# theori-io/nrsc5

Hardware: NVIDIA H100
Metric: cu8 I/Q Msamples/s (higher is better)
Workload: dtype u8/int16/f32

## Files before the change

### nrsc5_b200/csrc/common.cuh

```cuda
#pragma once
#include <cuda_runtime.h>
#include <stdint.h>

namespace nb {

constexpr int NFFT = 2048;
constexpr int NCP = 112;
constexpr int NSYM = NFFT + NCP;
constexpr int BLK = 32;
constexpr int NACQ = NSYM * (BLK + 1);
constexpr int LB0 = NFFT / 2 - 546;
constexpr int UB1 = NFFT / 2 + 546;
constexpr int PW = 19;
constexpr int MAXPART = 14;
constexpr int SIDE = MAXPART * PW + 1;
constexpr int NBINS = 2 * SIDE;
constexpr int PM_BLOCK = 23040;
constexpr int P1_LEN = 146176;
constexpr int P1_ENC = P1_LEN * 5 / 2;
constexpr int P1_VIT = P1_LEN * 3;
constexpr int P1_STEPS = P1_LEN + 64;
constexpr int PIDS_LEN = 80;
constexpr int P3_LEN = 4608;
constexpr int IV_N = 147456;
// ... 125 lines not shown
    int8_t *pm;
    short2 *ydec;
    float2 *acq_sums;
    float2 *tbuf;
    int8_t *vit_in;
    uint2 *vit_dec;
    uint32_t *p1_bits;
    uint2 *vspec, *vend;
    int *hstate, *tbend;
    uint32_t *v64_spec, *v64_end;
    int *v64_endstate;
    int8_t *px_ring[2];
    const uint32_t *iv_delay;
    const uint32_t *iv_delay_s;
    PxBufs xb[PX_GROUPS];
    uint8_t *log;
    const float *shape;
    const float2 *twid;
    const uint32_t *p1_lut;
    const uint8_t *pn;
    const uint32_t *pnw;
};

__device__ inline uint8_t *log_reserve(const DevPtrs &p, const EngineDims &d, int s, uint32_t type, uint32_t plen)
{
    StreamState &st = p.st[s];
    uint32_t need = 8 + ((plen + 3) & ~3u);
    if ((size_t)st.log_len + need > d.log_cap) {
        st.log_overflow = 1;
        return nullptr;
    }
    uint8_t *w = p.log + (size_t)s * d.log_cap + st.log_len;
    reinterpret_cast<uint32_t *>(w)[0] = type;
    reinterpret_cast<uint32_t *>(w)[1] = plen;
    st.log_len += need;
    return w + 8;
}

__device__ __forceinline__ void l2_enqueue(StreamState &st, int l2_on, unsigned off, unsigned lc, unsigned nbits)
{
    if (!l2_on) return;
    if (st.l2_n >= L2_QUEUE) {
        st.log_overflow = 1;
        return;
    }
    const int e = st.l2_n++;
    st.l2_off[e] = off;
    st.l2_lc[e] = lc;
    st.l2_nbits[e] = nbits;
// ... 39 lines not shown
```

### nrsc5_b200/csrc/engine.cu

```cuda
#include <cmath>
#include <cstdio>
#include <cstdlib>
#include <cstring>
#include <ctime>
#include <new>
#include <vector>

#include "../../include/nrsc5_b200.h"
#include "chan_feed.h"
#include "common.cuh"
#if defined(NB_EMU)
struct NvtxRange { explicit NvtxRange(const char *) {} };
#else
#include <nvtx3/nvToolsExt.h>
struct NvtxRange {
    explicit NvtxRange(const char *name) { nvtxRangePushA(name); }
    ~NvtxRange() { nvtxRangePop(); }
};
#endif
#include "rs.cuh"
#include "viterbi.cuh"
#include "viterbi_chunk.cuh"
#include "viterbi64.cuh"
#include "front.cuh"
// ... 129 lines not shown
    gf_tab_load(gf, t, P1_THREADS);
    if (t < 96) {
        unsigned v = frame ? __ldcg(frame + t) : 0;
        hdr[t] = (uint8_t)(__brev(v) >> 24);
    }
    __syncthreads();
    if (t < 32) {
        unsigned bit = 0;
        if (t < 24) {
            const unsigned i = 116176u + 1248u * t;
            const unsigned phys = (i & ~7u) + 7 - (i & 7);
            bit = ((p1_bit(bw, (int)phys) ^ (p.pnw[phys >> 5] >> (phys & 31))) & 1u) << (23 - t);
        }
        const unsigned pci = warp_xor(bit);
        const bool has_audio = (pci & 0xFFFFFC) != (0x3634CE & 0xFFFFFC);
        const int ok = has_audio ? rs8_fix_header_warp(gf, hdr, t) : 1;
        if (t == 0) {
            if (rec) *reinterpret_cast<float *>(rec) = (float)atomicAdd(&st.p1_errs, 0) / (float)P1_ENC;
            if (!ok) {
                if (st.state == ST_FINE && st.p1_lost_rec != 0xffffffffu) {
                    *reinterpret_cast<uint32_t *>(p.log + (size_t)s * d.log_cap + st.p1_lost_rec) = REC_LOST_SYNC;
                    st.state = ST_NONE;
                } else {
                    set_state(p, d, s, ST_NONE);
                }
            }
            if (st.p1_retry) st.p1_fallbacks++;
            st.p1_ready = 0;
            st.p1_slow = 0;
            st.p1_retry = 0;
            st.frames_done++;
        }
    }
}

__host__ __device__ inline VitcArgs p1_vitc_args(const DevPtrs &dp)
{
    VitcArgs a;
    a.vin = dp.vit_in;
    a.dec = dp.vit_dec;
    a.vspec = dp.vspec;
    a.vend = dp.vend;
    a.hstate = dp.hstate;
    a.tbend = dp.tbend;
    a.bitsw = dp.p1_bits;
    a.ready = &dp.st[0].p1_retry;
    a.slow = &dp.st[0].p1_slow;
// ... 954 lines not shown
static int publish_avail(nrsc5b_engine *e, int s, cudaStream_t on);

static int publish_pending(nrsc5b_engine *e, cudaStream_t on)
{
    for (int s = 0; s < e->dims.nstreams; s++)
        if (e->unpublished[s]) {
            int rc = publish_avail(e, s, on);
            if (rc) return rc;
            e->unpublished[s] = 0;
        }
    return 0;
}

static int publish_avail(nrsc5b_engine *e, int s, cudaStream_t on)
{
    if (e->avail_pos && (e->avail_pos & 4095) == 0) CK(cudaStreamSynchronize(on));
    long long *slot = e->avail_ring + (e->avail_pos++ & 4095);
    *slot = e->pushed[s];
    CK(cudaMemcpyAsync(reinterpret_cast<uint8_t *>(e->dp.st + s) + offsetof(StreamState, in_avail), slot, sizeof(*slot),
                       cudaMemcpyHostToDevice, on));
    return 0;
}

__global__ void k_trim_state(DevPtrs p, int s, long long drop, nbam::AmState *ast)
{
    p.st[s].start -= drop;
    p.st[s].in_avail -= 2 * drop;
    if (ast) ast[s].start -= drop;
}

static int trim_stream(nrsc5b_engine *e, int s)
{
    CK(cudaStreamSynchronize(e->copy_stream));
    CK(cudaStreamSynchronize(e->stream));
    StreamState st;
    CK(cudaMemcpy(&st, e->dp.st + s, sizeof(st), cudaMemcpyDeviceToHost));
    long long drop = (st.start - 64) & ~7LL;
    if (st.start < 72 || drop <= 0) return 0;
    const size_t off = 4 * (size_t)drop, have = 2 * (size_t)e->pushed[s];
    if (off >= have) return 0;
    const size_t rem = have - off;
    uint8_t *base = e->iq_owned + (size_t)s * e->dims.in_stride;
    if (!e->trim_scratch) {
        void *q = nullptr;
        if (cudaMalloc(&q, e->dims.in_stride) != cudaSuccess) return NRSC5B_ENOMEM;
        e->allocs.push_back(q);
// ... 125 lines not shown
    for (int s = 0; s < S; s++) e->pushed[s] += (long long)(nbytes / 2);
    e->direct_push = true;
    return NRSC5B_OK;
}

extern "C" int nrsc5b_push_cu8_device(nrsc5b_engine_t *e, int stream, const void *dev_buf, size_t nbytes)
{
    if (!e || stream < 0 || stream >= e->dims.nstreams || (nbytes & 3) || !e->iq_owned || e->am_ring) return NRSC5B_EINVAL;
    size_t off = (size_t)e->pushed[stream] * 2;
    if (off + nbytes > e->dims.in_stride) return NRSC5B_EFULL;
    CK(cudaMemcpyAsync(e->iq_owned + (size_t)stream * e->dims.in_stride + off, dev_buf, nbytes,
                       cudaMemcpyDeviceToDevice, e->stream));
    e->pushed[stream] += (long long)(nbytes / 2);
    e->direct_push = true;
    return publish_avail(e, stream, e->stream);
}

extern "C" int nrsc5b_attach_device_input(nrsc5b_engine_t *e, const void *dev_buf, size_t stride, size_t nbytes)
{
    if (!e || !dev_buf || (nbytes & 3) || nbytes > stride || e->am_ring) return NRSC5B_EINVAL;
    e->dp.iq = reinterpret_cast<const uint8_t *>(dev_buf);
    e->dims.in_stride = stride;
    e->direct_push = true;
    for (int s = 0; s < e->dims.nstreams; s++) {
        e->pushed[s] = (long long)(nbytes / 2);
        int rc = publish_avail(e, s, e->stream);
        if (rc) return rc;
    }
    return NRSC5B_OK;
}

int nbfeed_reserve(nrsc5b_engine_t *e, int device, int mode, const int *streams, int nch, long long nout, FeedTarget *t, long long *dst)
{
    if (!e || !t || !dst || nch <= 0 || nout < 0) return NRSC5B_EINVAL;
    if (e->cfg.mode != mode || !e->dims.cs16 || !e->iq_owned || e->dp.iq != e->iq_owned || device != e->cfg.device ||
        e->in_flight)
        return NRSC5B_EINVAL;
    const int S = e->dims.nstreams;
    if (!streams && nch > S) return NRSC5B_EINVAL;
    std::vector<uint8_t> seen(S, 0);
    for (int k = 0; k < nch; k++) {
        const int s = streams ? streams[k] : k;
        if (s < 0 || s >= S || seen[s]) return NRSC5B_EINVAL;
        seen[s] = 1;
    }
    const size_t need = 4 * (size_t)nout;
    bool full = false;
    for (int k = 0; k < nch; k++) {
        const int s = streams ? streams[k] : k;
        if ((size_t)e->pushed[s] * 2 + need <= e->dims.in_stride) continue;
        int rc = trim_stream(e, s);
// ... 932 lines not shown
```

### nrsc5_b200/csrc/front.cuh

```cuda
#pragma once
#include "pids_crc.cuh"
#include "common.cuh"
#include "fft.cuh"
#include "viterbi_pack.cuh"

namespace nb {

constexpr int FRONT_THREADS = 1024;
constexpr int TEAMS = FRONT_THREADS / 128;
constexpr int MAXREF = 15;
constexpr int IN_BYTES = 4 * NSYM + 28 + 16 + 16;
constexpr int IN_STRIDE = 8704;
constexpr int ACQ_TILE = 4096;

__device__ int g_dbg;

__constant__ int c_compat_mode[64];
__constant__ unsigned c_pn80[3];
__constant__ short c_bp_tap[32];

__device__ __forceinline__ float2 cmulf(float2 a, float2 b)
{
    return make_float2(a.x * b.x - a.y * b.y, a.x * b.y + a.y * b.x);
}
__device__ __forceinline__ float2 cexp_j(float a)
{
    float s, c;
    sincosf(a, &s, &c);
    return make_float2(c, s);
}

__device__ __forceinline__ int partitions_per_band(int psmi)
{
    switch (c_compat_mode[psmi & 63]) {
    case 2: return 11;
    case 3: return 12;
    case 5: case 6: case 11: return 14;
    default: return 10;
    }
}

__device__ void set_state(const DevPtrs &p, const EngineDims &d, int s, int ns)
{
    StreamState &st = p.st[s];
    if (st.state == ns) return;
    if (st.state == ST_FINE) log_reserve(p, d, s, REC_LOST_SYNC, 0);
    if (ns == ST_FINE) {
        float fo = (float)(((double)st.prev_angle - 2 * M_PI * st.cfo) * 744187.5 / (2 * M_PI * NFFT));
        uint8_t *w = log_reserve(p, d, s, REC_SYNC, 8);
        if (w) {
            reinterpret_cast<float *>(w)[0] = fo;
            reinterpret_cast<int *>(w)[1] = st.psmi;
        }
    }
    st.state = ns;
}

constexpr int DEMOD_RUN = 17;
constexpr int TEAM_SMEM = IN_STRIDE + NSYM * (int)sizeof(short2);
struct DemodSmem {
    float2 buf[TEAMS][TEAM_SMEM / sizeof(float2)];
};
static_assert(FFT_SMEM_ELEMS * sizeof(float2) <= TEAM_SMEM && TEAM_SMEM % 16 == 0, "a team's FFT buffer");
static_assert(DEMOD_RUN * FFT_THREADS >= NSYM && DEMOD_RUN % 2 == 1, "a symbol's runs");
struct PrepSmem {
    uint32_t words[ACQ_TILE + 40];
    short2 ytile[ACQ_TILE + 32];
    float2 sums[NSYM];
    float red_mag[FRONT_THREADS];
    int red_idx[FRONT_THREADS];
    float2 red_v[FRONT_THREADS];
};
// ... 35 lines not shown
    float wred[FRONT_THREADS / 32][2];
    float fb_w[2][MAXREF], fb_xy[2][MAXREF + 1];
    float4 rowc[EQ_ROWS];
    int ref_ok[2 * MAXREF], ref_bc[2 * MAXREF], ref_psmi[2 * MAXREF];
    bool px_on[2];
    long long px_T[2];
    uint8_t *soft_w;
    int do_search;
};
struct BlockSet {
    int samperr;
    int ok;
    float prev_angle, angle;
    float theta;
    float2 phase0, phase;
};
struct FrontSmem {
    float2 tw[FFT_TW];
    float2 nco[NSYM];
    float2 symphase[BLK];
    BlockSet blk;
    float2 zref[BLK][ZS];
    uint8_t ref_plan[128];
    union {
        DemodSmem demod;
        PrepSmem prep;
        Acq1Smem acq1;
        SyncSmem sync;
        PidsSmem pidsq[16];
    } u;
};

__device__ void pids_decode_warp(const DevPtrs &p, const EngineDims &d, int s, int e, PidsSmem &sm, int lane)
{
    const StreamState &st = p.st[s];
    const int bc = st.pids_bc[e];
    const int8_t *pmall = p.pm + (size_t)s * 16 * PM_BLOCK;
    const int8_t PMV[20] = { 10, 2, 18, 6, 14, 8, 16, 0, 12, 4, 11, 3, 19, 7, 15, 9, 17, 1, 13, 5 };
    for (int o = lane; o < PIDS_LEN * 3; o += 32) {
        int8_t v = 0;
        if (o % 6 != 5) {
            unsigned i = (unsigned)bc * 200 + (unsigned)(o - o / 6);
            unsigned part = (unsigned)PMV[i % 20];
            unsigned block = i / 200;
            unsigned k = (i / 20) % 10 + P1_ENC / 320;
            unsigned row = (k * 11) % 32, col = (k * 11 + k / 288) % 36;
            v = pmall[(block * 32 + row) * 720 + part * 36 + col];
        }
        sm.vit[o] = v;
    }
    __syncwarp();
    const int l = lane & 15;
    VitHalf<false> vh;
    vh.init(l);
    vitc_run<false>(vh, sm.vit, PIDS_LEN, PIDS_LEN + 64, 0, PIDS_LEN + 64, 0, sm.dec, lane < 16, l);
    __syncwarp();
    int v = (short)(vh.E & 0xffff), state = 2 * l;
    const int w1 = (short)(vh.O & 0xffff);
// ... 6 lines not shown
    for (int o = 8; o; o >>= 1) {
        const int ov = __shfl_xor_sync(0xffffffffu, v, o, 16), oi = __shfl_xor_sync(0xffffffffu, state, o, 16);
        if (ov > v || (ov == v && oi < state)) { v = ov; state = oi; }
    }
    if (lane == 0) {
        uint8_t pk[10];
        for (int i = 0; i < 10; i++) pk[i] = 0;
        for (int q = PIDS_LEN + 63; q >= 0; q--) {
            if (q >= 32 && q < 32 + PIDS_LEN) {
                const int i = q - 32;
                const int bit = ((state >> 5) & 1) ^ (int)((c_pn80[i >> 5] >> (i & 31)) & 1u);
                pk[i >> 3] |= (uint8_t)(bit << (7 - (i & 7)));
            }
            state = vitc_prev_head(state, sm.dec, q);
        }
        if (st.pids_rec[e] != 0xffffffffu) {
            uint8_t *w = p.log + (size_t)s * d.log_cap + st.pids_rec[e];
            for (int i = 0; i < 10; i++) w[i] = pk[i];
            w[10] = (uint8_t)pids_crc12_ok(pk);
        }
    }
}

__device__ void front_pids_flush(const DevPtrs &p, const EngineDims &d, int s, PidsSmem *sm, int t)
{
    StreamState &st = p.st[s];
    const int n = st.pids_pending, warp = t >> 5;
    if (warp < n) pids_decode_warp(p, d, s, warp, sm[warp], t & 31);
    __syncthreads();
    if (t == 0) st.pids_pending = 0;
}

constexpr int ACQ_RUN = 5;
static_assert(ACQ_RUN * FRONT_THREADS >= ACQ_TILE + 31, "a tile's runs");
template <int RUN>
__device__ __forceinline__ void acq_tile_input(const EngineDims &d, const uint32_t *words, short2 *ytile, const StreamState &st,
                                               int i0, int L, int t)
{
    const int kb = i0 == 0 ? 31 : 0;
    if (t < kb) ytile[t] = make_short2(st.bp_hist[t][0], st.bp_hist[t][1]);
    const int n = L + 31 - kb;
    if (d.cs16) {
        for (int k = kb + t; k < L + 31; k += FRONT_THREADS) {
            const uint32_t w = words[k + 7];
            ytile[k] = make_short2((short)(w & 0xffff), (short)(w >> 16));
        }
    } else if (RUN * t < n) {
        const int k = kb + min(RUN * t, n - RUN);
        halfband_run<RUN>(words + k, ytile + k);
    }
}
// ... 30 lines not shown
    double sn, cs;
    sincos((double)theta * (double)(NSYM * sym), &sn, &cs);
    symphase[sym] = cmul(phase0, make_float2((float)cs, (float)sn));
}

__device__ __forceinline__ void block_setup(BlockSet &b, const StreamState &st)
{
    const int adj = NSYM / 2 - b.samperr;
    float angle = b.prev_angle;
    angle = (float)((double)angle - 2 * M_PI * st.cfo);
    const float pre = (float)(-adj) * angle / (float)NFFT;
    const float2 ph = cmulf(st.phase, cexp_j(pre));
    const float theta = angle / (float)NFFT;
    double sn, cs;
    sincos((double)theta * (double)(NSYM * BLK), &sn, &cs);
    const float2 pe = cmulf(ph, make_float2((float)cs, (float)sn));
    const float nrm = sqrtf(pe.x * pe.x + pe.y * pe.y);
    b.angle = angle;
    b.theta = theta;
    b.phase0 = ph;
    b.phase = make_float2(pe.x / nrm, pe.y / nrm);
}

__device__ __forceinline__ void sync_adjust(const DevPtrs &p, int s, int adj, int t)
{
    if (adj == 0) return;
    float *cp = p.cphase + (size_t)s * NFFT;
    for (int i = t; i < SIDE; i += FRONT_THREADS) {
        const int bl = LB0 + i, bu = UB1 - i;
        cp[bl] = (float)((double)cp[bl] - (double)(adj * (bl - NFFT / 2) * 2) * M_PI / NFFT);
        cp[bu] = (float)((double)cp[bu] - (double)(adj * (bu - NFFT / 2) * 2) * M_PI / NFFT);
    }
}

__device__ __forceinline__ void block_commit(const DevPtrs &p, const EngineDims &d, int s, const BlockSet &b, int state_in)
{
    StreamState &st = p.st[s];
    st.phase0 = b.phase0;
    st.theta = b.theta;
    st.blk_samperr = b.samperr;
    st.blk_state_in = state_in;
    st.phase = b.phase;
    uint8_t *w = log_reserve(p, d, s, REC_BLOCK, 32);
    if (w) {
        int *wi = reinterpret_cast<int *>(w);
        float *wf = reinterpret_cast<float *>(w);
        wi[0] = state_in; wi[1] = b.samperr; wf[2] = b.angle; wf[3] = b.phase0.x; wf[4] = b.phase0.y; wi[5] = st.cfo;
        wi[6] = (int)(unsigned)(st.start & 0xffffffffLL);
        wi[7] = (int)(st.start >> 32);
    }
}

__device__ int front_prep_begin(const DevPtrs &p, const EngineDims &d, int s, int t)
{
    StreamState &st = p.st[s];
    __shared__ int sh_active;
    if (t == 0) {
        if (st.force_state >= 0) {
            set_state(p, d, s, st.force_state);
            st.force_state = -1;
        }
        const long long avail = *reinterpret_cast<volatile long long *>(&st.in_avail);
        int act = avail >= 2 * (st.start + NACQ);
        if (act && st.state == ST_FINE) {
            const int need = px_need_of(c_compat_mode[st.psmi & 63]);
            if (need & ~d.px_enabled) {
                atomicOr(&p.ctl->px_need, (unsigned)need);
                act = 0;
            }
        }
        st.active = act;
        sh_active = act ? (st.state == ST_FINE ? 1 : 2) : 0;
        if (act) atomicAdd(&p.ctl->progress, 1ull);
    }
    __syncthreads();
    const int mode = sh_active;
    __syncthreads();
    return mode;
}

__device__ void front_acq_tiles(const DevPtrs &p, const EngineDims &d, int s, PrepSmem &sm, int t, int rank, int nranks)
{
// ... 79 lines not shown
                }
            }
            __syncthreads();
        }
        if (t == 0) {
            const float2 w = cmulf(sm.red_v[0], cexp_j(-st.prev_angle));
            const float angle_diff = atan2f(w.y, w.x);
            const float factor = (st.prev_angle != 0.0f) ? 0.25f : 1.0f;
            const float angle = st.prev_angle + (angle_diff * factor);
            st.prev_angle = angle;
            b.prev_angle = angle;
            b.samperr = (sm.red_idx[0] + NSYM - 15) % NSYM;
            if (st.state == ST_NONE) st.state = ST_COARSE;
        }
    } else if (t == 0) {
        b.samperr = NSYM / 2 + st.samperr;
        st.samperr = 0;
        const float angle = st.prev_angle + (-st.angle);
        st.angle = 0;
        st.prev_angle = angle;
        b.prev_angle = angle;
    }
    __syncthreads();
    sync_adjust(p, s, NSYM / 2 - b.samperr, t);
    if (t == 0) {
        block_setup(b, st);
        block_commit(p, d, s, b, state_in);
    }
    __syncthreads();
    fill_nco(p, nco, b.theta, t);
    if (t >= FRONT_THREADS - BLK) fill_symphase(symphase, b.theta, b.phase0, t - (FRONT_THREADS - BLK));
    __syncthreads();
}

__device__ bool front_prep_single(const DevPtrs &p, const EngineDims &d, int s, Acq1Smem &sm, float2 *nco, float2 *symphase,
                                  BlockSet &b, int t)
{
    StreamState &st = p.st[s];
    __shared__ int sh_active;
    if (t == 0) {
        const int fs = st.force_state;
        const long long avail = *reinterpret_cast<volatile long long *>(&st.in_avail);
        const long long start = st.start;
        const int psmi = st.psmi;
        int state = st.state;
        if (fs >= 0) {
            set_state(p, d, s, fs);
            st.force_state = -1;
            state = fs;
        }
        int act = avail >= 2 * (start + NACQ);
        if (act && state == ST_FINE) {
            const int need = px_need_of(c_compat_mode[psmi & 63]);
            if (need & ~d.px_enabled) {
                atomicOr(&p.ctl->px_need, (unsigned)need);
                act = 0;
            }
        }
        st.active = act;
        sh_active = act ? (state == ST_FINE && b.ok ? 2 : 1) : 0;
        b.ok = 0;
        if (act) atomicAdd(&p.ctl->progress, 1ull);
    } else {
        fill_nco(p, nco, b.theta, t - 1, FRONT_THREADS - 1);
        if (t >= FRONT_THREADS - BLK) fill_symphase(symphase, b.theta, b.phase0, t - (FRONT_THREADS - BLK));
    }
    __syncthreads();
    if (!sh_active) return false;
    if (sh_active == 2) {
        sync_adjust(p, s, NSYM / 2 - b.samperr, t);
        if (t == 0) {
            st.samperr = 0;
            st.angle = 0;
            st.prev_angle = b.prev_angle;
            block_commit(p, d, s, b, ST_FINE);
        }
        return true;
    }

    const uint8_t *iq = p.iq + (size_t)s * d.in_stride;
    const int state_in = st.state;
    if (state_in != ST_FINE) {
        const long long start = st.start;
        constexpr int NT = BLK + 1;
        static_assert(NACQ == NT * NSYM, "the window is whole tiles");
        const int woff = (int)((start - 38) & 3);
        static_assert(NSYM % 4 == 0, "tiles start at the same word phase");
        const int nvec = (woff + NSYM + 38 + 3) / 4;
        auto fetch = [&](int T) {
            const long long w0 = start + (long long)T * NSYM - 38;
            const long long w0a = w0 & ~3LL;
            uint4 *dst = reinterpret_cast<uint4 *>(sm.words[T & 1]);
            for (int v = t; v < nvec; v += FRONT_THREADS) {
                const long long a = w0a + 4 * v;
                if (a >= 0) {
#if defined(NB_EMU)
                    dst[v] = *reinterpret_cast<const uint4 *>(iq + 4 * a);
#else
// ... 68 lines not shown
                }
            }
            __syncthreads();
        }
        if (t == 0) {
            const float2 w = cmulf(sm.red_v[0], cexp_j(-st.prev_angle));
            const float angle_diff = atan2f(w.y, w.x);
            const float factor = (st.prev_angle != 0.0f) ? 0.25f : 1.0f;
            const float angle = st.prev_angle + (angle_diff * factor);
            st.prev_angle = angle;
            b.prev_angle = angle;
            b.samperr = (sm.red_idx[0] + NSYM - 15) % NSYM;
            if (st.state == ST_NONE) st.state = ST_COARSE;
        }
    } else if (t == 0) {
        b.samperr = NSYM / 2 + st.samperr;
        st.samperr = 0;
        const float angle = st.prev_angle + (-st.angle);
        st.angle = 0;
        st.prev_angle = angle;
        b.prev_angle = angle;
    }
    __syncthreads();
    sync_adjust(p, s, NSYM / 2 - b.samperr, t);
    if (t == 0) {
        block_setup(b, st);
        block_commit(p, d, s, b, state_in);
    }
    __syncthreads();
    fill_nco(p, nco, b.theta, t);
    if (t >= FRONT_THREADS - BLK) fill_symphase(symphase, b.theta, b.phase0, t - (FRONT_THREADS - BLK));
    __syncthreads();
    return true;
}

__device__ __forceinline__ float2 sample_q15(short2 h)
{
    const float sc = 1.0f / 32767.0f;
    return make_float2((float)h.x * sc, (float)h.y * -sc);
}

__device__ void front_demod(const DevPtrs &p, const EngineDims &d, int s, int sym, DemodSmem &sm, const float2 *nco,
                            const float2 *symphase, const float2 *tw, float2 (*zref)[ZS], const uint8_t *ref_plan,
                            int half, int tl, long long start, int samperr)
{
    float2 *buf = sm.buf[half];
    uint8_t *in = reinterpret_cast<uint8_t *>(buf);
    const int bar = 1 + half;
    const long long base = start + samperr + (long long)NSYM * sym;
    const long long b0 = 4 * base - 28;
// ... 55 lines not shown

    float2 *dst = p.bins + ((size_t)s * BLK + sym) * NBINS;
    const unsigned plan = ref_plan[tl];
    float2 *zp = zref[sym] + (plan & 31u);
    const unsigned pk = plan >> 5;
    auto put = [&](int c, float2 v, unsigned k) {
        dst[c] = v;
        if (pk == k) *zp = v;
    };
#pragma unroll
    for (int h = 0; h < 2; h++) {
        const int q = tl + 128 * h;
        if (q >= 222) put(q - 222, cmul(out[h][5], sp), 4 * h);
        if (q <= 232) put(q + 34, cmul(out[h][6], sp), 4 * h + 1);
        if (q >= 24) put(q + 243, cmul(out[h][1], sp), 4 * h + 2);
        if (q <= 34) put(q + 499, cmul(out[h][2], sp), 4 * h + 3);
    }
}

__device__ __forceinline__ int ref_bin(int slot)
{
    return slot < MAXREF ? LB0 + PW * slot : UB1 - PW * (slot - MAXREF);
}

__device__ __forceinline__ float atan2_short(float y, float x)
{
    const float ax = fabsf(x), ay = fabsf(y);
    const float mx = fmaxf(ax, ay), mn = fminf(ax, ay);
    const float t = mx > 0.f ? __fdividef(mn, mx) : 0.f;
    const float z = t * t;
    float p = 0.0028340641874819994f;
    p = __fmaf_rn(p, z, -0.016005029901862144f);
    p = __fmaf_rn(p, z, 0.042587608098983765f);
    p = __fmaf_rn(p, z, -0.07495445758104324f);
    p = __fmaf_rn(p, z, 0.10636754333972931f);
    p = __fmaf_rn(p, z, -0.14202570915222168f);
    p = __fmaf_rn(p, z, 0.19992484152317047f);
    p = __fmaf_rn(p, z, -0.3333306610584259f);
    p = __fmaf_rn(p, z, 1.0f);
    float r = p * t;
    if (ay > ax) r = 1.57079637f - r;
    if (x < 0.f) r = 3.14159274f - r;
    return copysignf(r, y);
}

__device__ __forceinline__ void costas_row(float2 *z, float *phs, int zs, float &cfreq, float &cphase, int cfo, float alpha, float beta, bool FAST)
// ... 71 lines not shown
    }
    return -1;
}

__device__ __forceinline__ float half_pi_wrap(float a, float b)
{
    float dd = a - b;
    while ((double)dd > M_PI / 2) dd = (float)((double)dd - M_PI);
    while ((double)dd < -M_PI / 2) dd = (float)((double)dd + M_PI);
    return dd;
}

__device__ __forceinline__ int8_t soft_demap(float x, float mult)
{
    const float v = fmaxf(fminf(x, 1.0f), -1.0f) * mult;
    int r = __float2int_rz(v);
    const float f = v - (float)r;
    if (f >= 0.5f) r++;
    else if (f <= -0.5f) r--;
    return (int8_t)r;
}

template <bool CL>
__device__ void front_sync(const DevPtrs &p, const EngineDims &d, int s, SyncSmem &sm, float2 (*zref)[ZS], BlockSet &b, int t)
{
    StreamState &st = p.st[s];
    float *cfreq = p.cfreq + (size_t)s * NFFT;
    float *cphase = p.cphase + (size_t)s * NFFT;
    float2 *bins = p.bins + (size_t)s * BLK * NBINS;
    auto ldbin = [](const float2 *q) -> float2 { return CL ? __ldcg(q) : *q; };
    const float loop_bw = 0.05f, damping = 0.70710678f;
    const float denom = 1 + (2 * damping * loop_bw) + (loop_bw * loop_bw);
    const float alpha = (4 * damping * loop_bw) / denom, beta = (4 * loop_bw * loop_bw) / denom;

    int ppb = partitions_per_band(st.psmi);
    int nref = ppb + 1;
    long long sy0 = clock64();
    const bool sy_on = st.state == ST_FINE;
    auto sylap = [&](int k) {
        if (t == 0 && sy_on) {
            const long long c1 = clock64();
            st.sy_cyc[k] += (unsigned long long)(c1 - sy0);
            sy0 = c1;
        }
    };
    auto stage_eq = [&](int first, int stride) {
        const int rows = min(ppb, EQ_MAXPART) * (PW - 1), rows2 = 2 * rows;
        const int dn = stride / rows2, dr = stride - dn * rows2;
        int n = first / rows2, r = first - n * rows2;
#pragma unroll 4
        for (; n < BLK;) {
            const int sb = r >= rows, rr = sb ? r - rows : r;
            const int i = rr / (PW - 1);
            const int ci = sb == 0 ? rr + i + 1 : (NBINS - PW) + rr - (2 * PW - 1) * i;
            sm.eq[r][n] = ldbin(&bins[(size_t)n * NBINS + ci]);
            r += dr;
            n += dn;
            if (r >= rows2) { r -= rows2; n++; }
        }
    };
    const bool pre_staged = st.state == ST_FINE && !(g_dbg & 1);
    if (CL) {
        for (int i = t; i < ZS * BLK; i += FRONT_THREADS) {
            const int slot = i & (ZS - 1), n = i / ZS;
            const int ii = slot < MAXREF ? slot : slot - MAXREF;
            if (slot < 2 * MAXREF && ii < nref) zref[n][slot] = ldbin(&bins[(size_t)n * NBINS + compact_of_bin(ref_bin(slot))]);
        }
        __syncthreads();
    }
    sylap(0);
    if (t < 2 * MAXREF) {
        const int i = t < MAXREF ? t : t - MAXREF;
        if (i < nref) {
            const int b = ref_bin(t);
            float f = cfreq[b], ph = cphase[b];
            costas_row(&zref[0][t], &sm.phs[0][t], ZS, f, ph, 0, alpha, beta, !(g_dbg & 2));
            cfreq[b] = f;
            cphase[b] = ph;
            sm.cfq[t] = f;
            float sum = 0;
            for (int n = 0; n < BLK; n++) sum += fabsf(zref[n][t].x);
            sm.smag[t] = sum / BLK;
        }
    } else if (t >= 32 && pre_staged) {
        stage_eq(t - 32, FRONT_THREADS - 32);
    }
    __syncthreads();
    sylap(1);

    if (st.state == ST_COARSE) {
        if (t < 2 * MAXREF) {
            const int i = t < MAXREF ? t : t - MAXREF;
            sm.ref_ok[t] = 0;
            if (i < nref) {
                const float2 *z = &zref[0][t];
                const unsigned rsid = (unsigned)(30 - i) & 3;
                bool ok = true;
                unsigned raw = 0;
                for (int n = 0; n < BLK; n++) {
                    const int nbit = needle_bit(n, rsid);
                    const int pos = z[n * ZS].x > 0 ? 1 : 0;
// ... 8 lines not shown
            }
        }
        __syncthreads();
        if (t == 0) {
            unsigned good = 0;
            for (int r = 0; r < 2 * MAXREF; r++)
                if (sm.ref_ok[r]) good++;
            sm.do_search = 0;
            if (good >= 4) {
                int mbc = -1, mps = -1;
                for (int v = 0; v < 16; v++) {
                    unsigned nbc = 0, nps = 0;
                    for (int r = 0; r < 2 * MAXREF; r++) {
                        if (!sm.ref_ok[r]) continue;
                        nbc += sm.ref_bc[r] == v;
                        nps += sm.ref_psmi[r] == v;
                    }
                    if (nbc > good / 2) mbc = v;
                    if (nps > good / 2) mps = v;
                }
                if (mbc >= 0 && mps >= 0) {
                    st.bc = mbc;
                    st.psmi = mps;
                    set_state(p, d, s, ST_FINE);
                    l2_enqueue(st, d.l2, 0u, 0, 0);
                    st.started_pm = 0;
                    st.px_total[0] = st.px_total[1] = 0;
                    st.px_started[0] = st.px_started[1] = 0;
                }
            } else if (st.cfo_wait == 0) {
                sm.do_search = 1;
            } else {
                st.cfo_wait--;
            }
        }
        __syncthreads();
        if (sm.do_search) {
            for (int i = t; i < ZS * BLK; i += FRONT_THREADS) {
                const int slot = i & (ZS - 1), n = i / ZS;
                const int ii = slot < MAXREF ? slot : slot - MAXREF;
                if (slot < 2 * MAXREF && ii < nref) bins[(size_t)n * NBINS + compact_of_bin(ref_bin(slot))] = zref[n][slot];
            }
            for (int i = t; i < 76 * 22; i += FRONT_THREADS) sm.srch.offs[i / 22][i % 22] = -1;
            __syncthreads();
            constexpr int SB_BINS = 2 * PW * 2 + 10 * PW;
            constexpr int NSB = 2 * SB_BINS;
            float2 *snap = p.tbuf + (size_t)s * NACQ;
            float *sphs = reinterpret_cast<float *>(p.ydec + (size_t)s * NACQ);
            float fs[4], phsn[4];
            int cfo_of[4], nq = 0, ci = -1, b = 0;
            if (t < NSB) {
                const int upper = t >= SB_BINS;
                b = upper ? (UB1 - 10 * PW - 2 * PW) + (t - SB_BINS) : (LB0 - 2 * PW) + t;
                ci = compact_of_bin(b);
                float f = cfreq[b], ph = cphase[b];
                int ref_i[4];
                for (int step = 0; step <= 10; step++) {
                    const int i = upper ? step : 10 - step;
                    const int cfo = upper ? b - UB1 + PW * i : b - LB0 - PW * i;
                    if (cfo >= -2 * PW && cfo < 2 * PW && nq < 4) {
                        ref_i[nq] = i;
                        cfo_of[nq] = cfo;
                        nq++;
                    }
                }
                for (int q = 0; q < nq; q++) {
// ... 31 lines not shown
                if (win < (1 << 20)) {
                    st.keep_extra = ((BLK - sm.srch.verdict[win + 2 * PW]) % BLK) * NSYM;
                    st.cfo += win;
                    st.cfo_wait = 8;
                }
            }
            __syncthreads();
            if (t < NSB) {
                const int win = sm.srch.winner;
                int q = -1;
                for (int k = 0; k < nq; k++)
                    if (cfo_of[k] <= win) q = k;
                if (q >= 0) {
                    cfreq[b] = fs[q];
                    cphase[b] = phsn[q];
                    if (ci >= 0) {
                        const float2 *row = snap + (size_t)q * BLK * NSB + t;
                        for (int n = 0; n < BLK; n++) bins[(size_t)n * NBINS + ci] = row[(size_t)n * NSB];
                    }
                }
            }
        }
        __syncthreads();
    }

    if (st.state == ST_FINE) {
        for (int i = t; i < 2 * MAXREF * BLK; i += FRONT_THREADS) {
            const int slot = i >> 5, n = i & 31;
            const int ii = slot < MAXREF ? slot : slot - MAXREF;
            if (ii < nref) sm.eph[slot][n] = cexp_j(sm.phs[n][slot]);
        }
        const int bc = st.bc;
        int8_t *pm = p.pm + ((size_t)s * 16 + bc) * PM_BLOCK;
        const int rows = min(ppb, EQ_MAXPART) * (PW - 1), rows2 = 2 * rows;
        for (int r = t; r < rows2; r += FRONT_THREADS) {
            const int sb = r >= rows, rr = sb ? r - rows : r;
            const int i = rr / (PW - 1), k = rr - i * (PW - 1) + 1;
            int slot_lo, slot_hi;
            if (sb == 0) { slot_lo = i; slot_hi = i + 1; }
            else { slot_lo = MAXREF + i + 1; slot_hi = MAXREF + i; }
            sm.rowc[r] = make_float4((float)k * sm.smag[slot_hi], (float)(PW - k) * sm.smag[slot_lo],
                                     __int_as_float(slot_hi), __int_as_float(slot_lo));
        }
        sylap(2);
        if (!pre_staged) stage_eq(t, FRONT_THREADS);
        const int cm = c_compat_mode[st.psmi & 63];
// ... 130 lines not shown
                samperr = (float)((double)(samperr / (float)(ppb * 2) * (float)NFFT / (float)PW) * inv_2pi);
                for (int i = 0; i <= ppb; i++) {
                    float x;
                    x = (float)(LB0 + PW * i - NFFT / 2);
                    angle += sm.cfq[i]; sum_xy += sm.fb_xy[0][i]; sum_x2 += x * x;
                    x = (float)(UB1 - PW * i - NFFT / 2);
                    angle += sm.cfq[MAXREF + i]; sum_xy += sm.fb_xy[1][i]; sum_x2 += x * x;
                }
                samperr = (float)((double)samperr - (double)((sum_xy / sum_x2) * (float)NFFT) * inv_2pi * BLK);
                const int se = (int)roundf(samperr);
                st.samperr = se;
                angle /= (float)((ppb + 1) * 2);
                st.angle = angle;
                fb_angle = angle;
                if (!CL) {
                    b.samperr = NSYM / 2 + se;
                    b.prev_angle = st.prev_angle + (-angle);
                    block_setup(b, st);
                    b.ok = 1;
                }
            }
            fb_angle = __shfl_sync(0xffffffffu, fb_angle, 31);
            const int i = lane < MAXREF ? lane : lane - MAXREF;
            if (lane < 2 * MAXREF && i < nref) cfreq[ref_bin(lane)] = sm.cfq[lane] - fb_angle;
        } else if (t == 0) {
            st.err_lb += e_sb[0];
            st.err_ub += e_sb[1];
            if (++st.mer_cnt == 16) {
                const float signal = (float)(2 * BLK * (ppb * 18) * st.mer_cnt);
                uint8_t *w = log_reserve(p, d, s, REC_MER, 8);
                if (w) {
                    reinterpret_cast<float *>(w)[0] = 10 * log10f(signal / st.err_lb);
                    reinterpret_cast<float *>(w)[1] = 10 * log10f(signal / st.err_ub);
                }
                st.mer_cnt = 0;
                st.err_lb = 0;
                st.err_ub = 0;
            }
            if (d.emit_soft) {
                sm.soft_w = log_reserve(p, d, s, REC_SOFT_PM, 4 + PM_BLOCK);
                if (sm.soft_w) *reinterpret_cast<uint32_t *>(sm.soft_w) = (uint32_t)bc;
            }
            uint8_t *w = log_reserve(p, d, s, REC_PIDS, 11);
            const int e = st.pids_pending;
            st.pids_rec[e] = w ? (unsigned)(w - (p.log + (size_t)s * d.log_cap)) : 0xffffffffu;
            st.pids_bc[e] = bc;
            st.pids_pending = e + 1;
            if (bc == 0) st.started_pm = 1;
            unsigned lost_slot = 0xffffffffu;
            if (st.started_pm && bc == 15) {
                const unsigned len0 = st.log_len;
                uint8_t *bw = log_reserve(p, d, s, REC_BER, 4);
                uint8_t *fw = bw ? log_reserve(p, d, s, REC_FRAME, 8 + P1_LEN / 8) : nullptr;
                if (!fw) { st.log_len = len0; bw = nullptr; }
                st.p1_rec = (bw && fw) ? (unsigned)(bw - (p.log + (size_t)s * d.log_cap)) : 0xffffffffu;
                if (fw) {
                    reinterpret_cast<uint32_t *>(fw)[0] = 0;
                    reinterpret_cast<uint32_t *>(fw)[1] = P1_LEN;
                    uint8_t *lw = log_reserve(p, d, s, REC_PAD, 0);
                    if (lw) lost_slot = (unsigned)(lw - 8 - (p.log + (size_t)s * d.log_cap));
                }
                st.p1_lost_rec = lost_slot;
                l2_enqueue(st, d.l2, st.p1_rec != 0xffffffffu ? st.p1_rec + 4 + 8 + 8 : 0xffffffffu, 0, P1_LEN);
                st.p1_ready = 1;
            }
#pragma unroll
            for (int g = 0; g < PX_GROUPS; g++) {
                const PxGroup x = px_group(g);
                if (!(x.modes >> cm & 1)) continue;
                if ((bc & 1) == 0) st.px_started[x.ring] = 1;
                if (!st.px_started[x.ring]) continue;
                st.px_total[x.ring] += x.len;
                const long long k0 = st.px_total[x.ring] - 2 * x.len;
                if ((bc & 1) && k0 >= 32 * x.len && st.xq_pending[g] < P3_SLOTS) {
                    uint8_t *fw = log_reserve(p, d, s, REC_FRAME, 8 + x.len / 8);
                    const int e = st.xq_pending[g];
                    st.xq_k0[g][e] = k0;
                    st.xq_rec[g][e] = fw ? (unsigned)(fw - (p.log + (size_t)s * d.log_cap)) : 0xffffffffu;
                    if (fw) {
                        reinterpret_cast<uint32_t *>(fw)[0] = x.lc;
                        reinterpret_cast<uint32_t *>(fw)[1] = x.len;
                    }
                    l2_enqueue(st, d.l2, fw ? st.xq_rec[g][e] + 8 : 0xffffffffu, x.lc, x.len);
                    st.xq_pending[g] = e + 1;
                }
            }
            if (lost_slot != 0xffffffffu && st.log_len == lost_slot + 8) {
                st.log_len = lost_slot;
                st.p1_lost_rec = 0xffffffffu;
            }
            st.bc = (bc + 1) % 16;
        }
        __syncthreads();
        if (d.emit_soft && sm.soft_w)
            for (int o = t; o < PM_BLOCK; o += FRONT_THREADS) sm.soft_w[4 + o] = (uint8_t)pm[o];
    }
    if (t == 0) {
        const int keep = NSYM + (NSYM / 2 - st.blk_samperr) + st.keep_extra;
// ... 4 lines not shown
    sylap(5);
}

__device__ __forceinline__ void cluster_barrier()
{
#if defined(NB_EMU)
#else
    asm volatile("barrier.cluster.arrive.release.aligned;\n\tbarrier.cluster.wait.acquire.aligned;" ::: "memory");
#endif
}

template <bool CL>
__global__ void __launch_bounds__(FRONT_THREADS, 1) k_stream(DevPtrs p, EngineDims d, int max_blocks, int last_pass)
{
#if defined(NB_EMU)
    unsigned char *front_smem_raw = emu::dyn_smem();
#else
    extern __shared__ __align__(16) unsigned char front_smem_raw[];
#endif
    FrontSmem &sm = *reinterpret_cast<FrontSmem *>(front_smem_raw);
    const int t = threadIdx.x, team = t >> 7, tl = t & 127;
    const int C = CL ? d.cluster : 1;
    const int s = (int)blockIdx.x / C, rank = (int)blockIdx.x % C;
    StreamState &st = p.st[s];
    for (int i = t; i < FFT_TW; i += FRONT_THREADS) sm.tw[i] = __ldg(&p.twid[i]);
    if (t < 128) {
        unsigned m = 0xffu;
        for (int h = 0; h < 2; h++) {
            const int q = t + 128 * h;
            const int c[4] = { q >= 222 ? q - 222 : -1, q <= 232 ? q + 34 : -1, q >= 24 ? q + 243 : -1, q <= 34 ? q + 499 : -1 };
            for (int k = 0; k < 4; k++) {
                if (c[k] < 0) continue;
                const int slot = c[k] < SIDE ? (c[k] % PW == 0 ? c[k] / PW : -1)
                                             : ((NBINS - 1 - c[k]) % PW == 0 ? MAXREF + (NBINS - 1 - c[k]) / PW : -1);
                if (slot >= 0) m = (unsigned)(4 * h + k) << 5 | (unsigned)slot;
            }
        }
        sm.ref_plan[t] = (uint8_t)m;
    }
    if (t == 0) {
        sm.blk.ok = 0;
        sm.blk.theta = 0.f;
        sm.blk.phase0 = make_float2(0.f, 0.f);
    }
    __syncthreads();

    const bool owner = !CL || rank == 0;
    if (max_blocks > 16) max_blocks = 16;
    if (owner && t == 0) {
        for (int g = 0; g < PX_GROUPS; g++) st.xq_pending[g] = 0;
    }
    __syncthreads();
    for (int nb = 0;; nb++) {
        long long c0 = clock64();
        auto lap = [&](int ph) {
            if (owner && t == 0) {
                const long long c1 = clock64();
                st.ph_cyc[ph] += (unsigned long long)(c1 - c0);
                st.ph_n[ph]++;
                c0 = c1;
            }
        };
        int mode = 0;
        if (!CL) {
            if (nb < max_blocks && !st.p1_ready) mode = front_prep_single(p, d, s, sm.u.acq1, sm.nco, sm.symphase, sm.blk, t) ? 1 : 0;
            if (mode == 0) break;
        } else {
            if (owner) {
                if (nb < max_blocks && !st.p1_ready) mode = front_prep_begin(p, d, s, t);
                if (mode == 1) front_prep_finish(p, d, s, sm.u.prep, sm.nco, sm.symphase, sm.blk, t, 1);
            }
            if (owner && t == 0) {
                st.blk_go = mode;
                __threadfence();
            }
            cluster_barrier();
            if (!owner) mode = __ldcg(&st.blk_go);
            if (mode == 0) break;
            if (mode == 2) {
                front_acq_tiles(p, d, s, sm.u.prep, t, rank, C);
                __threadfence();
                cluster_barrier();
                front_acq_corr(p, s, t, rank, C);
                __threadfence();
                cluster_barrier();
                if (owner) {
                    front_prep_finish(p, d, s, sm.u.prep, sm.nco, sm.symphase, sm.blk, t, 2);
                    __threadfence();
// ... 1 lines not shown
                cluster_barrier();
            }
        }
        lap(st.blk_state_in == ST_FINE ? 2 : 1);
        const long long start = CL ? __ldcg(&st.start) : st.start;
        const int samperr = CL ? __ldcg(&st.blk_samperr) : sm.blk.samperr;
        if (CL && !owner) {
            const float theta = __ldcg(&st.theta);
            fill_nco(p, sm.nco, theta, t);
            if (t >= FRONT_THREADS - BLK) fill_symphase(sm.symphase, theta, __ldcg(&st.phase0), t - (FRONT_THREADS - BLK));
            __syncthreads();
        }
#pragma unroll 1
        for (int pass = 0; pass < BLK / (TEAMS * C); pass++)
            front_demod(p, d, s, (pass * C + rank) * TEAMS + team, sm.u.demod, sm.nco, sm.symphase, sm.tw, sm.zref, sm.ref_plan,
                            team, tl, start, samperr);
        if (CL) {
            __threadfence();
            cluster_barrier();
        }
        if (CL && !owner) continue;
        __syncthreads();
        lap(3);
        front_sync<CL>(p, d, s, sm.u.sync, sm.zref, sm.blk, t);
        __syncthreads();
        lap(st.blk_state_in == ST_FINE ? 4 : 5);
    }
    if (CL && !owner) return;
    __syncthreads();
    if (st.pids_pending) {
        const long long c0 = clock64();
        front_pids_flush(p, d, s, sm.u.pidsq, t);
        if (t == 0) {
            st.ph_cyc[0] += (unsigned long long)(clock64() - c0);
            st.ph_n[0]++;
        }
    }
    if (t == 0) {
        StreamBrief b;
        b.start = st.start;
        b.state = st.state;
        b.bc = st.bc;
        b.p1_ready = st.p1_ready;
        b.pad_ = 0;
        p.brief[s] = b;
        const long long avail = *reinterpret_cast<volatile long long *>(&st.in_avail);
        if (last_pass && avail >= 2 * (st.start + NACQ)) atomicAdd(&p.ctl->more, 1u);
    }
}

}
```

Before: 180,400.

## Cache per-stream state and Costas loop arrays in shared memory for single-CTA path

```diff
diff --git a/nrsc5_b200/csrc/common.cuh b/nrsc5_b200/csrc/common.cuh
--- a/nrsc5_b200/csrc/common.cuh
+++ b/nrsc5_b200/csrc/common.cuh
@@ -171,9 +171,8 @@
     const uint32_t *pnw;
 };
 
-__device__ inline uint8_t *log_reserve(const DevPtrs &p, const EngineDims &d, int s, uint32_t type, uint32_t plen)
-{
-    StreamState &st = p.st[s];
+__device__ inline uint8_t *log_reserve(const DevPtrs &p, const EngineDims &d, int s, StreamState &st, uint32_t type, uint32_t plen)
+{
     uint32_t need = 8 + ((plen + 3) & ~3u);
     if ((size_t)st.log_len + need > d.log_cap) {
         st.log_overflow = 1;
diff --git a/nrsc5_b200/csrc/engine.cu b/nrsc5_b200/csrc/engine.cu
--- a/nrsc5_b200/csrc/engine.cu
+++ b/nrsc5_b200/csrc/engine.cu
@@ -175,7 +175,7 @@
                     *reinterpret_cast<uint32_t *>(p.log + (size_t)s * d.log_cap + st.p1_lost_rec) = REC_LOST_SYNC;
                     st.state = ST_NONE;
                 } else {
-                    set_state(p, d, s, ST_NONE);
+                    set_state(p, d, s, st, ST_NONE);
                 }
             }
             if (st.p1_retry) st.p1_fallbacks++;
@@ -1176,6 +1176,12 @@
     return 0;
 }
 
+__global__ void k_publish_all(DevPtrs p, int S, long long avail)
+{
+    const int s = (int)(blockIdx.x * blockDim.x + threadIdx.x);
+    if (s < S) p.st[s].in_avail = avail;
+}
+
 __global__ void k_trim_state(DevPtrs p, int s, long long drop, nbam::AmState *ast)
 {
     p.st[s].start -= drop;
@@ -1347,11 +1353,11 @@
     e->dp.iq = reinterpret_cast<const uint8_t *>(dev_buf);
     e->dims.in_stride = stride;
     e->direct_push = true;
-    for (int s = 0; s < e->dims.nstreams; s++) {
-        e->pushed[s] = (long long)(nbytes / 2);
-        int rc = publish_avail(e, s, e->stream);
-        if (rc) return rc;
-    }
+    const int S = e->dims.nstreams;
+    for (int s = 0; s < S; s++) e->pushed[s] = (long long)(nbytes / 2);
+    k_publish_all<<<(S + 127) / 128, 128, 0, e->stream>>>(e->dp, S, (long long)(nbytes / 2));
+    e->stats.kernel_launches += 1;
+    CK(cudaGetLastError());
     return NRSC5B_OK;
 }
 
diff --git a/nrsc5_b200/csrc/front.cuh b/nrsc5_b200/csrc/front.cuh
--- a/nrsc5_b200/csrc/front.cuh
+++ b/nrsc5_b200/csrc/front.cuh
@@ -40,14 +40,13 @@
     }
 }
 
-__device__ void set_state(const DevPtrs &p, const EngineDims &d, int s, int ns)
-{
-    StreamState &st = p.st[s];
+__device__ void set_state(const DevPtrs &p, const EngineDims &d, int s, StreamState &st, int ns)
+{
     if (st.state == ns) return;
-    if (st.state == ST_FINE) log_reserve(p, d, s, REC_LOST_SYNC, 0);
+    if (st.state == ST_FINE) log_reserve(p, d, s, st, REC_LOST_SYNC, 0);
     if (ns == ST_FINE) {
         float fo = (float)(((double)st.prev_angle - 2 * M_PI * st.cfo) * 744187.5 / (2 * M_PI * NFFT));
-        uint8_t *w = log_reserve(p, d, s, REC_SYNC, 8);
+        uint8_t *w = log_reserve(p, d, s, st, REC_SYNC, 8);
         if (w) {
             reinterpret_cast<float *>(w)[0] = fo;
             reinterpret_cast<int *>(w)[1] = st.psmi;
@@ -129,6 +128,8 @@
     BlockSet blk;
     float2 zref[BLK][ZS];
     uint8_t ref_plan[128];
+    StreamState st;
+    float kfreq[NBINS], kphase[NBINS];
     union {
         DemodSmem demod;
         PrepSmem prep;
@@ -137,10 +138,15 @@
         PidsSmem pidsq[16];
     } u;
 };
-
-__device__ void pids_decode_warp(const DevPtrs &p, const EngineDims &d, int s, int e, PidsSmem &sm, int lane)
-{
-    const StreamState &st = p.st[s];
+static_assert(sizeof(FrontSmem) <= 227 * 1024, "k_stream's shared memory fits an SM's 227 KB");
+
+__device__ __forceinline__ int bin_of_compact(int c)
+{
+    return c < SIDE ? LB0 + c : UB1 - (NBINS - 1 - c);
+}
+
+__device__ void pids_decode_warp(const DevPtrs &p, const EngineDims &d, int s, const StreamState &st, int e, PidsSmem &sm, int lane)
+{
     const int bc = st.pids_bc[e];
     const int8_t *pmall = p.pm + (size_t)s * 16 * PM_BLOCK;
     const int8_t PMV[20] = { 10, 2, 18, 6, 14, 8, 16, 0, 12, 4, 11, 3, 19, 7, 15, 9, 17, 1, 13, 5 };
@@ -193,11 +199,10 @@
     }
 }
 
-__device__ void front_pids_flush(const DevPtrs &p, const EngineDims &d, int s, PidsSmem *sm, int t)
-{
-    StreamState &st = p.st[s];
+__device__ void front_pids_flush(const DevPtrs &p, const EngineDims &d, int s, StreamState &st, PidsSmem *sm, int t)
+{
     const int n = st.pids_pending, warp = t >> 5;
-    if (warp < n) pids_decode_warp(p, d, s, warp, sm[warp], t & 31);
+    if (warp < n) pids_decode_warp(p, d, s, st, warp, sm[warp], t & 31);
     __syncthreads();
     if (t == 0) st.pids_pending = 0;
 }
@@ -274,26 +279,25 @@
     b.phase = make_float2(pe.x / nrm, pe.y / nrm);
 }
 
-__device__ __forceinline__ void sync_adjust(const DevPtrs &p, int s, int adj, int t)
+__device__ __forceinline__ void sync_adjust(float *lo, float *hi, int adj, int t)
 {
     if (adj == 0) return;
-    float *cp = p.cphase + (size_t)s * NFFT;
     for (int i = t; i < SIDE; i += FRONT_THREADS) {
         const int bl = LB0 + i, bu = UB1 - i;
-        cp[bl] = (float)((double)cp[bl] - (double)(adj * (bl - NFFT / 2) * 2) * M_PI / NFFT);
-        cp[bu] = (float)((double)cp[bu] - (double)(adj * (bu - NFFT / 2) * 2) * M_PI / NFFT);
-    }
-}
-
-__device__ __forceinline__ void block_commit(const DevPtrs &p, const EngineDims &d, int s, const BlockSet &b, int state_in)
-{
-    StreamState &st = p.st[s];
+        lo[i] = (float)((double)lo[i] - (double)(adj * (bl - NFFT / 2) * 2) * M_PI / NFFT);
+        hi[-i] = (float)((double)hi[-i] - (double)(adj * (bu - NFFT / 2) * 2) * M_PI / NFFT);
+    }
+}
+
+__device__ __forceinline__ void block_commit(const DevPtrs &p, const EngineDims &d, int s, StreamState &st, const BlockSet &b,
+                                             int state_in)
+{
     st.phase0 = b.phase0;
     st.theta = b.theta;
     st.blk_samperr = b.samperr;
     st.blk_state_in = state_in;
     st.phase = b.phase;
-    uint8_t *w = log_reserve(p, d, s, REC_BLOCK, 32);
+    uint8_t *w = log_reserve(p, d, s, st, REC_BLOCK, 32);
     if (w) {
         int *wi = reinterpret_cast<int *>(w);
         float *wf = reinterpret_cast<float *>(w);
@@ -309,7 +313,7 @@
     __shared__ int sh_active;
     if (t == 0) {
         if (st.force_state >= 0) {
-            set_state(p, d, s, st.force_state);
+            set_state(p, d, s, st, st.force_state);
             st.force_state = -1;
         }
         const long long avail = *reinterpret_cast<volatile long long *>(&st.in_avail);
@@ -435,10 +439,11 @@
         b.prev_angle = angle;
     }
     __syncthreads();
-    sync_adjust(p, s, NSYM / 2 - b.samperr, t);
+    float *cp = p.cphase + (size_t)s * NFFT;
+    sync_adjust(cp + LB0, cp + UB1, NSYM / 2 - b.samperr, t);
     if (t == 0) {
         block_setup(b, st);
-        block_commit(p, d, s, b, state_in);
+        block_commit(p, d, s, st, b, state_in);
     }
     __syncthreads();
     fill_nco(p, nco, b.theta, t);
@@ -446,19 +451,18 @@
     __syncthreads();
 }
 
-__device__ bool front_prep_single(const DevPtrs &p, const EngineDims &d, int s, Acq1Smem &sm, float2 *nco, float2 *symphase,
-                                  BlockSet &b, int t)
-{
-    StreamState &st = p.st[s];
+__device__ bool front_prep_single(const DevPtrs &p, const EngineDims &d, int s, StreamState &st, float *kphase, Acq1Smem &sm,
+                                  float2 *nco, float2 *symphase, BlockSet &b, int t)
+{
     __shared__ int sh_active;
     if (t == 0) {
         const int fs = st.force_state;
-        const long long avail = *reinterpret_cast<volatile long long *>(&st.in_avail);
+        const long long avail = *reinterpret_cast<volatile long long *>(&p.st[s].in_avail);
         const long long start = st.start;
         const int psmi = st.psmi;
         int state = st.state;
         if (fs >= 0) {
-            set_state(p, d, s, fs);
+            set_state(p, d, s, st, fs);
             st.force_state = -1;
             state = fs;
         }
@@ -481,12 +485,12 @@
     __syncthreads();
     if (!sh_active) return false;
     if (sh_active == 2) {
-        sync_adjust(p, s, NSYM / 2 - b.samperr, t);
+        sync_adjust(kphase, kphase + NBINS - 1, NSYM / 2 - b.samperr, t);
         if (t == 0) {
             st.samperr = 0;
             st.angle = 0;
             st.prev_angle = b.prev_angle;
-            block_commit(p, d, s, b, ST_FINE);
+            block_commit(p, d, s, st, b, ST_FINE);
         }
         return true;
     }
@@ -601,10 +605,10 @@
         b.prev_angle = angle;
     }
     __syncthreads();
-    sync_adjust(p, s, NSYM / 2 - b.samperr, t);
+    sync_adjust(kphase, kphase + NBINS - 1, NSYM / 2 - b.samperr, t);
     if (t == 0) {
         block_setup(b, st);
-        block_commit(p, d, s, b, state_in);
+        block_commit(p, d, s, st, b, state_in);
     }
     __syncthreads();
     fill_nco(p, nco, b.theta, t);
@@ -706,6 +710,10 @@
 {
     return slot < MAXREF ? LB0 + PW * slot : UB1 - PW * (slot - MAXREF);
 }
+__device__ __forceinline__ int ref_compact(int slot)
+{
+    return slot < MAXREF ? PW * slot : NBINS - 1 - PW * (slot - MAXREF);
+}
 
 __device__ __forceinline__ float atan2_short(float y, float x)
 {
@@ -823,11 +831,13 @@
 }
 
 template <bool CL>
-__device__ void front_sync(const DevPtrs &p, const EngineDims &d, int s, SyncSmem &sm, float2 (*zref)[ZS], BlockSet &b, int t)
-{
-    StreamState &st = p.st[s];
+__device__ void front_sync(const DevPtrs &p, const EngineDims &d, int s, StreamState &st, float *kfreq, float *kphase,
+                           SyncSmem &sm, float2 (*zref)[ZS], BlockSet &b, int t)
+{
     float *cfreq = p.cfreq + (size_t)s * NFFT;
     float *cphase = p.cphase + (size_t)s * NFFT;
+    float *rfreq = CL ? cfreq : kfreq, *rphase = CL ? cphase : kphase;
+    auto rix = [](int slot) { return CL ? ref_bin(slot) : ref_compact(slot); };
     float2 *bins = p.bins + (size_t)s * BLK * NBINS;
     auto ldbin = [](const float2 *q) -> float2 { return CL ? __ldcg(q) : *q; };
     const float loop_bw = 0.05f, damping = 0.70710678f;
@@ -873,11 +883,11 @@
     if (t < 2 * MAXREF) {
         const int i = t < MAXREF ? t : t - MAXREF;
         if (i < nref) {
-            const int b = ref_bin(t);
-            float f = cfreq[b], ph = cphase[b];
+            const int b = rix(t);
+            float f = rfreq[b], ph = rphase[b];
             costas_row(&zref[0][t], &sm.phs[0][t], ZS, f, ph, 0, alpha, beta, !(g_dbg & 2));
-            cfreq[b] = f;
-            cphase[b] = ph;
+            rfreq[b] = f;
+            rphase[b] = ph;
             sm.cfq[t] = f;
             float sum = 0;
             for (int n = 0; n < BLK; n++) sum += fabsf(zref[n][t].x);
@@ -932,7 +942,7 @@
                 if (mbc >= 0 && mps >= 0) {
                     st.bc = mbc;
                     st.psmi = mps;
-                    set_state(p, d, s, ST_FINE);
+                    set_state(p, d, s, st, ST_FINE);
                     l2_enqueue(st, d.l2, 0u, 0, 0);
                     st.started_pm = 0;
                     st.px_total[0] = st.px_total[1] = 0;
@@ -952,6 +962,11 @@
                 if (slot < 2 * MAXREF && ii < nref) bins[(size_t)n * NBINS + compact_of_bin(ref_bin(slot))] = zref[n][slot];
             }
             for (int i = t; i < 76 * 22; i += FRONT_THREADS) sm.srch.offs[i / 22][i % 22] = -1;
+            if (!CL)
+                for (int c = t; c < NBINS; c += FRONT_THREADS) {
+                    cfreq[bin_of_compact(c)] = kfreq[c];
+                    cphase[bin_of_compact(c)] = kphase[c];
+                }
             __syncthreads();
             constexpr int SB_BINS = 2 * PW * 2 + 10 * PW;
             constexpr int NSB = 2 * SB_BINS;
@@ -1029,6 +1044,11 @@
             }
         }
         __syncthreads();
+        if (!CL && sm.do_search)
+            for (int c = t; c < NBINS; c += FRONT_THREADS) {
+                kfreq[c] = cfreq[bin_of_compact(c)];
+                kphase[c] = cphase[bin_of_compact(c)];
+            }
     }
 
     if (st.state == ST_FINE) {
@@ -1205,13 +1225,13 @@
             }
             fb_angle = __shfl_sync(0xffffffffu, fb_angle, 31);
             const int i = lane < MAXREF ? lane : lane - MAXREF;
-            if (lane < 2 * MAXREF && i < nref) cfreq[ref_bin(lane)] = sm.cfq[lane] - fb_angle;
+            if (lane < 2 * MAXREF && i < nref) rfreq[rix(lane)] = sm.cfq[lane] - fb_angle;
         } else if (t == 0) {
             st.err_lb += e_sb[0];
             st.err_ub += e_sb[1];
             if (++st.mer_cnt == 16) {
                 const float signal = (float)(2 * BLK * (ppb * 18) * st.mer_cnt);
-                uint8_t *w = log_reserve(p, d, s, REC_MER, 8);
+                uint8_t *w = log_reserve(p, d, s, st, REC_MER, 8);
                 if (w) {
                     reinterpret_cast<float *>(w)[0] = 10 * log10f(signal / st.err_lb);
                     reinterpret_cast<float *>(w)[1] = 10 * log10f(signal / st.err_ub);
@@ -1221,10 +1241,10 @@
                 st.err_ub = 0;
             }
             if (d.emit_soft) {
-                sm.soft_w = log_reserve(p, d, s, REC_SOFT_PM, 4 + PM_BLOCK);
+                sm.soft_w = log_reserve(p, d, s, st, REC_SOFT_PM, 4 + PM_BLOCK);
                 if (sm.soft_w) *reinterpret_cast<uint32_t *>(sm.soft_w) = (uint32_t)bc;
             }
-            uint8_t *w = log_reserve(p, d, s, REC_PIDS, 11);
+            uint8_t *w = log_reserve(p, d, s, st, REC_PIDS, 11);
             const int e = st.pids_pending;
             st.pids_rec[e] = w ? (unsigned)(w - (p.log + (size_t)s * d.log_cap)) : 0xffffffffu;
             st.pids_bc[e] = bc;
@@ -1233,14 +1253,14 @@
             unsigned lost_slot = 0xffffffffu;
             if (st.started_pm && bc == 15) {
                 const unsigned len0 = st.log_len;
-                uint8_t *bw = log_reserve(p, d, s, REC_BER, 4);
-                uint8_t *fw = bw ? log_reserve(p, d, s, REC_FRAME, 8 + P1_LEN / 8) : nullptr;
+                uint8_t *bw = log_reserve(p, d, s, st, REC_BER, 4);
+                uint8_t *fw = bw ? log_reserve(p, d, s, st, REC_FRAME, 8 + P1_LEN / 8) : nullptr;
                 if (!fw) { st.log_len = len0; bw = nullptr; }
                 st.p1_rec = (bw && fw) ? (unsigned)(bw - (p.log + (size_t)s * d.log_cap)) : 0xffffffffu;
                 if (fw) {
                     reinterpret_cast<uint32_t *>(fw)[0] = 0;
                     reinterpret_cast<uint32_t *>(fw)[1] = P1_LEN;
-                    uint8_t *lw = log_reserve(p, d, s, REC_PAD, 0);
+                    uint8_t *lw = log_reserve(p, d, s, st, REC_PAD, 0);
                     if (lw) lost_slot = (unsigned)(lw - 8 - (p.log + (size_t)s * d.log_cap));
                 }
                 st.p1_lost_rec = lost_slot;
@@ -1256,7 +1276,7 @@
                 st.px_total[x.ring] += x.len;
                 const long long k0 = st.px_total[x.ring] - 2 * x.len;
                 if ((bc & 1) && k0 >= 32 * x.len && st.xq_pending[g] < P3_SLOTS) {
-                    uint8_t *fw = log_reserve(p, d, s, REC_FRAME, 8 + x.len / 8);
+                    uint8_t *fw = log_reserve(p, d, s, st, REC_FRAME, 8 + x.len / 8);
                     const int e = st.xq_pending[g];
                     st.xq_k0[g][e] = k0;
                     st.xq_rec[g][e] = fw ? (unsigned)(fw - (p.log + (size_t)s * d.log_cap)) : 0xffffffffu;
@@ -1307,7 +1327,20 @@
     const int t = threadIdx.x, team = t >> 7, tl = t & 127;
     const int C = CL ? d.cluster : 1;
     const int s = (int)blockIdx.x / C, rank = (int)blockIdx.x % C;
-    StreamState &st = p.st[s];
+    StreamState &st = CL ? p.st[s] : sm.st;
+    float *cfreq = p.cfreq + (size_t)s * NFFT, *cphase = p.cphase + (size_t)s * NFFT;
+    constexpr int ST_WORDS = (int)(sizeof(StreamState) / sizeof(unsigned long long));
+    static_assert(sizeof(StreamState) % sizeof(unsigned long long) == 0 && offsetof(StreamState, in_avail) == 0,
+                  "the state is copied in 8-byte words, and in_avail is its first");
+    if (!CL) {
+        const unsigned long long *gw = reinterpret_cast<const unsigned long long *>(&p.st[s]);
+        unsigned long long *sw = reinterpret_cast<unsigned long long *>(&sm.st);
+        for (int i = t; i < ST_WORDS; i += FRONT_THREADS) sw[i] = gw[i];
+        for (int c = t; c < NBINS; c += FRONT_THREADS) {
+            sm.kfreq[c] = cfreq[bin_of_compact(c)];
+            sm.kphase[c] = cphase[bin_of_compact(c)];
+        }
+    }
     for (int i = t; i < FFT_TW; i += FRONT_THREADS) sm.tw[i] = __ldg(&p.twid[i]);
     if (t < 128) {
         unsigned m = 0xffu;
@@ -1348,7 +1381,7 @@
         };
         int mode = 0;
         if (!CL) {
-            if (nb < max_blocks && !st.p1_ready) mode = front_prep_single(p, d, s, sm.u.acq1, sm.nco, sm.symphase, sm.blk, t) ? 1 : 0;
+            if (nb < max_blocks && !st.p1_ready) mode = front_prep_single(p, d, s, st, sm.kphase, sm.u.acq1, sm.nco, sm.symphase, sm.blk, t) ? 1 : 0;
             if (mode == 0) break;
         } else {
             if (owner) {
@@ -1396,7 +1429,7 @@
         if (CL && !owner) continue;
         __syncthreads();
         lap(3);
-        front_sync<CL>(p, d, s, sm.u.sync, sm.zref, sm.blk, t);
+        front_sync<CL>(p, d, s, st, sm.kfreq, sm.kphase, sm.u.sync, sm.zref, sm.blk, t);
         __syncthreads();
         lap(st.blk_state_in == ST_FINE ? 4 : 5);
     }
@@ -1404,7 +1437,7 @@
     __syncthreads();
     if (st.pids_pending) {
         const long long c0 = clock64();
-        front_pids_flush(p, d, s, sm.u.pidsq, t);
+        front_pids_flush(p, d, s, st, sm.u.pidsq, t);
         if (t == 0) {
             st.ph_cyc[0] += (unsigned long long)(clock64() - c0);
             st.ph_n[0]++;
@@ -1418,9 +1451,19 @@
         b.p1_ready = st.p1_ready;
         b.pad_ = 0;
         p.brief[s] = b;
-        const long long avail = *reinterpret_cast<volatile long long *>(&st.in_avail);
+        const long long avail = *reinterpret_cast<volatile long long *>(&p.st[s].in_avail);
         if (last_pass && avail >= 2 * (st.start + NACQ)) atomicAdd(&p.ctl->more, 1u);
     }
-}
-
-}
+    if (!CL) {
+        __syncthreads();
+        const unsigned long long *sw = reinterpret_cast<const unsigned long long *>(&sm.st);
+        unsigned long long *gw = reinterpret_cast<unsigned long long *>(&p.st[s]);
+        for (int i = 1 + t; i < ST_WORDS; i += FRONT_THREADS) gw[i] = sw[i];
+        for (int c = t; c < NBINS; c += FRONT_THREADS) {
+            cfreq[bin_of_compact(c)] = sm.kfreq[c];
+            cphase[bin_of_compact(c)] = sm.kphase[c];
+        }
+    }
+}
+
+}
```

Result: faster. 197,800 (median of 6 runs) (+9.7%).
